# PersiaML/PERSIA

Measured on NVIDIA B200. Metric: samples/sec (Criteo-1TB-shape DLRM sparse path, 26 slots, dim128), higher is better.
Workload: dtype f32

## Files before the change

### persia_b200/csrc/pb_kernels.cuh

```cuda
#pragma once
#include <atomic>

#include "pb_common.cuh"

namespace pb {

struct SlotsDev {
  uint64_t prefix[PB_MAX_SLOTS];
  uint32_t occ_off[PB_MAX_SLOTS + 1];
  uint8_t sqrt_scaling[PB_MAX_SLOTS];
  uint32_t n_slots;
  uint64_t spacing;
  uint32_t spacing_bits;
  uint32_t uniform;
};

struct GradsDev {
  const void* ptr[PB_MAX_SLOTS];
  float inv_scale[PB_MAX_SLOTS];
  uint8_t do_scale[PB_MAX_SLOTS];
  const float* adam_pow;
  uint8_t pow_idx[PB_MAX_SLOTS];
};

constexpr uint32_t PB_GIANT_MIN = 1024;
constexpr uint32_t PB_HUGE_MIN = 256;
constexpr uint32_t PB_WARM_MAX = 32;
enum {
  BC_ITEMS = 0,
  BC_COLD,
  BC_WARM,
  BC_HOT,
  BC_SEG,
  BC_HUGE,
  BC_HOTW,
  BC_GIANT,
  BC_PEER = 8,
  BC_NEXT = 24,
  BC_COUNT = BC_NEXT + 2 * PB_MAX_SLOTS
};
struct BatchDev {
  DCell* set;
  uint32_t* occ_set;
  uint32_t* item_cell;
  uint32_t* seg_occ;
  uint2* cold;
  uint4* warm;
  uint4* hot;
  uint32_t* hot_bits;
  uint32_t hot_words;
  uint32_t hot_cap;
  uint32_t giant_cap;
  uint32_t* cnt;
  uint32_t n;
};

enum { XC_FLAG_SIGN = 0, XC_FLAG_ROW, XC_FLAG_GRAD, XC_COUNT, XC_WORDS };
constexpr uint32_t PB_MAX_RANKS = 16;
constexpr uint32_t PB_ADAM_KEYS = 256;
struct __align__(16) UCell {
  uint32_t row;
  uint32_t mask;
  uint32_t k[PB_MAX_RANKS];
  uint32_t pad[2];
};
struct XchgDev {
  uint64_t base[PB_MAX_RANKS];
  uint64_t off_sign, off_row, off_grad, off_gok;
  uint32_t R, rank, cap, row_f32;
  uint32_t* epoch;
  uint32_t* waited;
  uint32_t* own_row;
  uint32_t* own_cnt;
  uint32_t* err;
  UCell* ucell;
  uint32_t* uwin;
  uint32_t ucells;
  const uint64_t* akeys;
  uint32_t n_akeys;
  uint64_t amask;
  uint32_t* apresent;
  float* apow;
};

struct ReduceArgs {
  BatchDev b;
  const uint32_t* occ_outrow;
  const uint32_t* row_off;
  const uint32_t* tick_ptr;
  const uint32_t* nan_tick;
  float* vw_stage;
  uint32_t batch, round, quiet_miss;
  uint32_t round_mask[PB_MAX_SLOTS / 32];
  XchgDev x;
};

struct RawCell {
  uint64_t key;
  uint32_t first;
  uint32_t rank;
};
struct RawWork {
  RawCell* set;
  uint32_t set_mask;
  uint32_t* occ_set;
  uint32_t* flag;
  uint32_t* rank;
  uint32_t* tiles;
  uint32_t* distinct_cell;
  uint32_t* counts;
};

void launch_fill_cells(Cell* cells, uint64_t n, cudaStream_t st);
void launch_fill_set(DCell* set, uint64_t n, cudaStream_t st);
void launch_begin_batch(const TableDev& t, uint32_t* ctx_tick, uint32_t* batch_cnt, cudaStream_t st, bool bump = true);
void launch_probe(int mode, bool prefix, const TableDev& t, const HyperDev& hy, const OptimDev& op, const SlotsDev& sl,
                  const uint64_t* ids, uint32_t n, uint32_t* occ_cell, cudaStream_t st);
void launch_gather(const TableDev& t, const uint32_t* occ_cell, uint32_t n_out, float* out, cudaStream_t st);
void launch_dedup(const SlotsDev& sl, const BatchDev& b, const uint64_t* ids, cudaStream_t st);
void launch_probe_items(bool training, const TableDev& t, const HyperDev& hy, const OptimDev& op, const SlotsDev& sl,
                        const BatchDev& b, cudaStream_t st);
void launch_gather_items(const TableDev& t, const SlotsDev& sl, const BatchDev& b, const uint32_t* row_off,
// ... 72 lines not shown
```

### persia_b200/csrc/pb_reduce.cu

```cuda
#include <cstdlib>

#include "pb_optim.cuh"

namespace pb {

struct ItemSrc {
  const void* gbase;
  uint32_t slot_row0;
  float inv_scale;
  bool do_scale, do_sqrt, plain;
};

__device__ __forceinline__ ItemSrc item_src(const SlotsDev& sl, const GradsDev& gr, const ReduceArgs& a, uint32_t slot) {
  ItemSrc s;
  s.gbase = gr.ptr[slot];
  s.slot_row0 = slot * a.batch;
  s.inv_scale = gr.inv_scale[slot];
  s.do_scale = gr.do_scale[slot];
  s.do_sqrt = sl.sqrt_scaling[slot];
  s.plain = !a.occ_outrow && !s.do_scale && !s.do_sqrt;
  return s;
}

__device__ __forceinline__ uint32_t occ_out_row(const ReduceArgs& a, uint32_t occ) {
// ... 186 lines not shown
      } else {
        send_item<VEC, F16>(t, sl, gr, a, row, slot, cnt, lane, G, [&](uint32_t k) { return srt[k]; });
      }
      continue;
    }
    if (slot_dead(dead, slot)) continue;
    if (row >= t.capacity) {
      if (lane == 0 && !a.quiet_miss) atomicAdd(&t.counters[CTR_GRAD_MISS], 1u);
      continue;
    }
    float* stage = a.vw_stage ? a.vw_stage + (size_t)(n_cold + w) * t.dim : nullptr;
    step_item<VEC, F16, KIND>(t, op, hy, sl, gr, a, row, slot, cnt, lane, G, gmask, stage, [&](uint32_t k) { return srt[k]; });
  }
}

template <int VEC, bool F16, int KIND, bool SEND>
__global__ void __launch_bounds__(256) k_reduce_cold(TableDev t, OptimDev op, HyperDev hy, SlotsDev sl, GradsDev gr,
                                                     ReduceArgs a, uint32_t G) {
  __shared__ uint32_t dead[PB_MAX_SLOTS / 32];
  const uint32_t n_cold = a.b.cnt[BC_COLD];
  if (blockIdx.x * (blockDim.x / G) >= n_cold) return;
  build_dead_mask(dead, gr, a, sl.n_slots);
  const uint32_t lane = threadIdx.x % G, wl = threadIdx.x & 31;
  const uint32_t gmask = (G == 32) ? 0xffffffffu : (((1u << G) - 1u) << (wl / G * G));
  const uint32_t nvec = t.dim / VEC;
  for (uint32_t w = blockIdx.x * (blockDim.x / G) + threadIdx.x / G; w < n_cold; w += gridDim.x * (blockDim.x / G)) {
    const uint2 d = a.b.cold[w];
    const uint32_t slot = slot_of_occ(sl, d.y);
    const ItemSrc src = item_src(sl, gr, a, slot);
    const uint32_t orow = occ_out_row(a, d.y);
    const GradPrep prep = grad_prep(src, a, orow);
    const size_t gelem = (size_t)(orow - src.slot_row0) * t.dim;
    if (SEND) {
      if (d.x == ROW_NONE) continue;
      const bool off = slot_dead(dead, slot);
      if (lane == 0) *send_gok_ptr(a.x, d.x) = off ? 0u : 1u;
      if (off) continue;
      float* dst = send_grad_ptr(a.x, d.x, t.dim);
      for (uint32_t c = lane; c < nvec; c += G) {
        float g[VEC], acc[VEC];
        load_grad_elems<VEC, F16>(g, src.gbase, gelem, c * VEC);
#pragma unroll
        for (int q = 0; q < VEC; ++q) acc[q] = 0.0f;
        add_prepared<VEC>(acc, g, prep, src.plain);
        store_vec<VEC>(dst + c * VEC, acc);
      }
      continue;
    }
    if (slot_dead(dead, slot)) continue;
    if (d.x >= t.capacity) {
      if (lane == 0 && !a.quiet_miss) atomicAdd(&t.counters[CTR_GRAD_MISS], 1u);
      continue;
    }
    if (KIND == PB_OPT_ADAGRAD_VW) {
      const uint32_t occ = d.y;
      step_item<VEC, F16, KIND>(t, op, hy, sl, gr, a, d.x, slot, 1u, lane, G, gmask, a.vw_stage + (size_t)w * t.dim,
                                [&](uint32_t) { return occ; });
      continue;
    }
    float* prow = t.rows + (size_t)d.x * t.stride;
    StepCtx sc;
    sc.vw_state = sc.r1 = sc.r2 = 0.0f;
    if (KIND == PB_OPT_ADAM) sc = step_ctx(prow, t, op, gr, slot);
    for (uint32_t c = lane; c < nvec; c += G) {
      RowElems<KIND, VEC> rc;
      float g[VEC], acc[VEC];
      rc.load(prow, c * VEC, t, op);
      load_grad_elems<VEC, F16>(g, src.gbase, gelem, c * VEC);
#pragma unroll
      for (int q = 0; q < VEC; ++q) acc[q] = 0.0f;
      add_prepared<VEC>(acc, g, prep, src.plain);
      rc.step(c * VEC, acc, t, op, hy, sc);
      rc.store(prow, c * VEC, t, op);
    }
  }
}

constexpr uint32_t HOT_WIN = 8192;
constexpr uint32_t HOT_WORDS = HOT_WIN / 32;
constexpr uint32_t HOT_THREADS = 256;
constexpr uint32_t HOT_WARPS = HOT_THREADS / 32;
constexpr uint32_t HOT_MAX_SLOTS = 8;
constexpr uint32_t HOT_COLS = 512;
constexpr uint32_t WAIT_SPINS = 1u << 22;

__device__ __forceinline__ uint32_t smem_u32(const void* p) { return (uint32_t)__cvta_generic_to_shared(p); }
__device__ __forceinline__ void mbar_init(uint32_t bar, uint32_t count) {
  asm volatile("mbarrier.init.shared::cta.b64 [%0], %1;" ::"r"(bar), "r"(count) : "memory");
}
__device__ __forceinline__ void mbar_arrive(uint32_t bar) {
  asm volatile("mbarrier.arrive.shared::cta.b64 _, [%0];" ::"r"(bar) : "memory");
}
__device__ __forceinline__ bool mbar_wait(uint32_t bar, uint32_t parity) {
  for (uint32_t spins = 0; spins < WAIT_SPINS; ++spins) {
    uint32_t done;
    asm volatile(
        "{\n\t.reg .pred p;\n\t"
        "mbarrier.try_wait.parity.shared::cta.b64 p, [%1], %2;\n\t"
        "selp.u32 %0, 1, 0, p;\n\t}"
        : "=r"(done)
        : "r"(bar), "r"(parity)
        : "memory");
    if (done) return true;
  }
  return false;
}

__device__ __forceinline__ unsigned long long globaltimer_ns() {
  unsigned long long now;
  asm volatile("mov.u64 %0, %%globaltimer;" : "=l"(now));
  return now;
}
__device__ __forceinline__ bool mbar_test(uint32_t bar, uint32_t parity) {
  uint32_t done;
  asm volatile(
      "{\n\t.reg .pred p;\n\t"
      "mbarrier.test_wait.parity.shared::cta.b64 p, [%1], %2;\n\t"
      "selp.u32 %0, 1, 0, p;\n\t}"
      : "=r"(done)
      : "r"(bar), "r"(parity)
      : "memory");
  return done;
}

__device__ __forceinline__ __half2 clamp_h2(__half2 v) {
  const __half2 lim = __floats2half2_rn(65504.0f, 65504.0f);
  return __hmin2(__hmax2(v, __hneg2(lim)), lim);
}

struct HotGeom {
  uint32_t cols;
  uint32_t stride;
  uint32_t R;
  uint32_t R1;
  uint32_t S;
  uint32_t rowbytes;
  uint32_t lean;
  uint32_t CH;
  uint32_t vec;
  uint32_t vshift;
};

template <bool F16, bool POW2>
__device__ __forceinline__ void produce_vec(float* slot, const HotGeom& g, const ItemSrc& src, uint32_t my_row, float my_f,
                                            uint32_t nv, uint32_t col0, uint32_t dim, uint32_t lane) {
  constexpr uint32_t EV = F16 ? 8u : 4u;
  const unsigned char* gcol = reinterpret_cast<const unsigned char*>(src.gbase) + (size_t)col0 * (F16 ? 2u : 4u);
  const uint32_t rowbytes = dim * (F16 ? 2u : 4u);
  const uint32_t nvr = g.cols / EV, total = g.R1 * nvr, nv4 = (nv + 3u) & ~3u;
  uint4 raw[8];
#pragma unroll
  for (int j = 0; j < 8; ++j) {
    const uint32_t v = (uint32_t)j * 32u + lane;
    const uint32_t r = POW2 ? v >> g.vshift : v / nvr, c = POW2 ? v & (nvr - 1u) : v % nvr;
    const uint32_t grow = __shfl_sync(0xffffffffu, my_row, r & 31u);
    raw[j] = make_uint4(0u, 0u, 0u, 0u);
    if (v < total && r < nv) raw[j] = __ldg(reinterpret_cast<const uint4*>(gcol + (size_t)grow * rowbytes + c * 16u));
  }
  const bool prep = src.do_scale || src.do_sqrt;
#pragma unroll
  for (int j = 0; j < 8; ++j) {
    const uint32_t v = (uint32_t)j * 32u + lane;
    const uint32_t r = POW2 ? v >> g.vshift : v / nvr, c = POW2 ? v & (nvr - 1u) : v % nvr;
    float f = 1.0f;
    if (prep) f = __shfl_sync(0xffffffffu, my_f, r & 31u);
    if (v >= total || r >= nv4) continue;
    float x[EV];
    if constexpr (F16) {
      const __half2* h = reinterpret_cast<const __half2*>(&raw[j]);
#pragma unroll
      for (int q = 0; q < 4; ++q) {
        float2 y = __half22float2(clamp_h2(h[q]));
        x[2 * q] = y.x;
        x[2 * q + 1] = y.y;
      }
    } else {
      x[0] = __uint_as_float(raw[j].x); x[1] = __uint_as_float(raw[j].y);
      x[2] = __uint_as_float(raw[j].z); x[3] = __uint_as_float(raw[j].w);
    }
    if (prep) {
      if (src.do_scale) {
#pragma unroll
        for (uint32_t q = 0; q < EV; ++q) x[q] = __fmul_rn(x[q], src.inv_scale);
      }
      if (src.do_sqrt) {
#pragma unroll
        for (uint32_t q = 0; q < EV; ++q) x[q] = __fmul_rn(x[q], f);
      }
    }
    float4* dst = reinterpret_cast<float4*>(slot + (size_t)r * g.stride + c * EV);
    dst[0] = make_float4(x[0], x[1], x[2], x[3]);
    if constexpr (F16) dst[1] = make_float4(x[4], x[5], x[6], x[7]);
  }
}

template <bool F16>
__device__ __forceinline__ void produce_chunk(float* slot, const HotGeom& g, const ItemSrc& src, const ReduceArgs& a,
                                              const uint16_t* sorted, uint32_t k0, uint32_t nv, uint32_t wbase,
                                              uint32_t col0, uint32_t dim, uint32_t lane) {
  uint32_t my_row = 0;
  float my_f = 0.0f;
  if (lane < nv) {
    const uint32_t orow = occ_out_row(a, wbase + sorted[k0 + lane]);
    my_row = orow - src.slot_row0;
    my_f = src.do_sqrt ? grad_prep(src, a, orow).sqrt_f : 1.0f;
  }
  if (g.vec) {
    if (g.vshift < 32u) produce_vec<F16, true>(slot, g, src, my_row, my_f, nv, col0, dim, lane);
    else produce_vec<F16, false>(slot, g, src, my_row, my_f, nv, col0, dim, lane);
  } else {
    const unsigned char* gbytes = reinterpret_cast<const unsigned char*>(src.gbase);
    const uint32_t nv4 = min(g.R1, (nv + 3u) & ~3u), total = nv4 * g.cols;
    for (uint32_t i0 = 0; i0 < total; i0 += 32u) {
      const uint32_t i = i0 + lane;
      const bool ok = i < total;
      const uint32_t r = ok ? i / g.cols : 0u, c = ok ? i % g.cols : 0u;
      const uint32_t grow = __shfl_sync(0xffffffffu, my_row, r);
      const float f = __shfl_sync(0xffffffffu, my_f, r);
      if (!ok) continue;
      float x = 0.0f;
      if (r < nv) {
        const size_t e = (size_t)grow * dim + col0 + c;
        x = F16 ? clamp_f16(__half2float(reinterpret_cast<const __half*>(gbytes)[e])) : reinterpret_cast<const float*>(gbytes)[e];
        if (src.do_scale) x = __fmul_rn(x, src.inv_scale);
        if (src.do_sqrt) x = __fmul_rn(x, f);
      }
      slot[(size_t)r * g.stride + c] = x;
    }
  }
}

__device__ __forceinline__ void lean_load(uint4 (&raw)[8], const HotGeom& g, const unsigned char* gcol0, const uint16_t* sorted,
                                          uint32_t nv, uint32_t lane) {
  const uint32_t nvr_mask = (1u << g.vshift) - 1u;
  const uint32_t r0 = lane >> g.vshift, rstep = 32u >> g.vshift;
  const unsigned char* gc = gcol0 + (lane & nvr_mask) * 16u;
#pragma unroll
  for (int j = 0; j < 8; ++j) {
    const uint32_t r = (uint32_t)j * rstep + r0;
    raw[j] = make_uint4(0u, 0u, 0u, 0u);
    if (r < nv) raw[j] = __ldg(reinterpret_cast<const uint4*>(gc + (size_t)sorted[r] * g.rowbytes));
  }
}
template <bool F16>
__device__ __forceinline__ void lean_store(float* slot, const uint4 (&raw)[8], const HotGeom& g, uint32_t nv, uint32_t lane) {
  constexpr uint32_t EV = F16 ? 8u : 4u;
  const uint32_t nvr_mask = (1u << g.vshift) - 1u, nv4 = (nv + 3u) & ~3u;
  const uint32_t r0 = lane >> g.vshift, rstep = 32u >> g.vshift;
  float* sc = slot + (lane & nvr_mask) * EV;
#pragma unroll
  for (int j = 0; j < 8; ++j) {
    const uint32_t r = (uint32_t)j * rstep + r0;
    if (r >= nv4) continue;
    float4* dst = reinterpret_cast<float4*>(sc + (size_t)r * g.stride);
    if constexpr (F16) {
      const __half2* h = reinterpret_cast<const __half2*>(&raw[j]);
      const float2 y0 = __half22float2(clamp_h2(h[0])), y1 = __half22float2(clamp_h2(h[1]));
      const float2 y2 = __half22float2(clamp_h2(h[2])), y3 = __half22float2(clamp_h2(h[3]));
      dst[0] = make_float4(y0.x, y0.y, y1.x, y1.y);
      dst[1] = make_float4(y2.x, y2.y, y3.x, y3.y);
    } else {
      dst[0] = make_float4(__uint_as_float(raw[j].x), __uint_as_float(raw[j].y), __uint_as_float(raw[j].z), __uint_as_float(raw[j].w));
    }
  }
}

template <int EPL, int RB>
__device__ __forceinline__ void chain_block(float (&acc)[EPL], const float* rp, uint32_t stride) {
  float v[RB][EPL];
#pragma unroll
  for (int u = 0; u < RB; ++u) RowElems<-1, EPL>::template ld<EPL>(rp + (size_t)u * stride, v[u]);
#pragma unroll
  for (int u = 0; u < RB; ++u) {
#pragma unroll
    for (int q = 0; q < EPL; ++q) acc[q] = __fadd_rn(acc[q], v[u][q]);
  }
}

template <int EPL, bool F16, bool SEND>
__global__ void __launch_bounds__(HOT_THREADS, 1) k_reduce_hot(TableDev t, OptimDev op, HyperDev hy, SlotsDev sl, GradsDev gr,
                                                              ReduceArgs a, HotGeom geo, unsigned long long* trace) {
  extern __shared__ __align__(128) unsigned char smem_raw[];
  __shared__ uint32_t dead[PB_MAX_SLOTS / 32];
  __shared__ uint32_t s_item, s_nwin;
  __shared__ uint32_t bitmap[HOT_WORDS], wpre[HOT_WORDS];
  __shared__ uint16_t sorted[HOT_WIN];
  __shared__ __align__(8) uint64_t bars[2 * HOT_MAX_SLOTS];
  float* ring = reinterpret_cast<float*>(smem_raw);
  float* vstage = ring + (size_t)geo.S * geo.R * geo.stride;
  const uint32_t tid = threadIdx.x, warp = tid >> 5, lane = tid & 31;
  const uint32_t CH = geo.CH, PW = min(HOT_WARPS - CH, geo.S);
  if (tid == 0) {
    for (uint32_t s = 0; s < HOT_MAX_SLOTS; ++s) {
      mbar_init(smem_u32(bars + s), 32u);
      mbar_init(smem_u32(bars + HOT_MAX_SLOTS + s), 32u * CH);
    }
    asm volatile("fence.mbarrier_init.release.cluster;" ::: "memory");
  }
  build_dead_mask(dead, gr, a, sl.n_slots);
  const uint32_t full0 = smem_u32(bars), empty0 = smem_u32(bars + HOT_MAX_SLOTS);
  const uint32_t n_giant = a.b.cnt[BC_GIANT], n_huge = a.b.cnt[BC_HUGE];
  const uint32_t n_hot = a.b.cnt[BC_HOT] + n_huge + n_giant;
  uint32_t* next = a.b.cnt + BC_NEXT + PB_MAX_SLOTS + a.round;
  const uint32_t n_pass = (t.dim + HOT_COLS - 1u) / HOT_COLS;
  uint32_t it = 0;
  bool failed = false;
  for (;;) {
    __syncthreads();
    if (tid == 0) s_item = atomicAdd(next, 1u);
    __syncthreads();
    const uint32_t h = s_item;
    if (h >= n_hot) break;
    if (trace && tid == 0) trace[8 * h] = globaltimer_ns();
    const uint4 d = a.b.hot[h < n_giant ? a.b.hot_cap - 1u - h
                                        : (h < n_giant + n_huge ? a.b.hot_cap - 1u - a.b.giant_cap - (h - n_giant) : h - n_giant - n_huge)];
    const uint32_t row = d.x, cnt = d.z, slot = d.w;
    const bool bm_mode = d.y >> 31;
    const uint32_t base = d.y & 0x7FFFFFFFu;
    const uint32_t lo = sl.occ_off[slot], hi = sl.occ_off[slot + 1];
    bool skip = false;
    if (SEND) {
      skip = row == ROW_NONE || slot_dead(dead, slot);
      if (row != ROW_NONE && tid == 0) *send_gok_ptr(a.x, row) = slot_dead(dead, slot) ? 0u : 1u;
    } else {
      skip = slot_dead(dead, slot) || row >= t.capacity;
      if (!slot_dead(dead, slot) && row >= t.capacity && tid == 0 && !a.quiet_miss) atomicAdd(&t.counters[CTR_GRAD_MISS], 1u);
    }
    if (skip) {
      if (bm_mode)
        for (uint32_t w = tid; w < (hi - lo + 31u) / 32u; w += HOT_THREADS) a.b.hot_bits[base + w] = 0u;
      continue;
    }
    const ItemSrc src = item_src(sl, gr, a, slot);
    float* prow = SEND ? send_grad_ptr(a.x, row, t.dim) : t.rows + (size_t)row * t.stride;
    StepCtx sc;
    sc.vw_state = sc.r1 = sc.r2 = 0.0f;
    if (!SEND) sc = step_ctx(prow, t, op, gr, slot);
    for (uint32_t pass = 0; pass < n_pass; ++pass) {
      const uint32_t col0 = pass * HOT_COLS;
      HotGeom g = geo;
      g.cols = min(geo.cols, t.dim - col0);
      if (g.cols != geo.cols) g.vec = g.lean = 0;
      const bool lean = g.lean && src.plain;
      const uint32_t e0 = col0 + (warp * 32u + lane) * EPL;
      const bool own = warp < CH && e0 < t.dim;
      float acc[EPL];
#pragma unroll
      for (int q = 0; q < EPL; ++q) acc[q] = 0.0f;
      for (uint32_t wbase = lo; wbase < hi; wbase += HOT_WIN) {
        const uint32_t wend = min(hi, wbase + HOT_WIN);
        const uint32_t n_words = (wend - wbase + 31u) / 32u;
        if (bm_mode) {
          uint32_t* gw = a.b.hot_bits + base + (wbase - lo) / 32u;
          for (uint32_t w = tid; w < HOT_WORDS; w += HOT_THREADS) {
            bitmap[w] = w < n_words ? gw[w] : 0u;
            if (w < n_words && pass + 1 == n_pass) gw[w] = 0u;
          }
        } else {
          for (uint32_t w = tid; w < HOT_WORDS; w += HOT_THREADS) bitmap[w] = 0u;
          __syncthreads();
          for (uint32_t k0 = tid; k0 < cnt; k0 += 4 * HOT_THREADS) {
            uint32_t p[4];
#pragma unroll
            for (int u = 0; u < 4; ++u) p[u] = k0 + u * HOT_THREADS < cnt ? a.b.seg_occ[base + k0 + u * HOT_THREADS] : 0xFFFFFFFFu;
#pragma unroll
            for (int u = 0; u < 4; ++u)
              if (p[u] >= wbase && p[u] < wend) atomicOr(&bitmap[(p[u] - wbase) >> 5], 1u << ((p[u] - wbase) & 31u));
          }
        }
        __syncthreads();
        if (warp == 0) {
          uint32_t c[HOT_WORDS / 32], sum = 0;
#pragma unroll
          for (uint32_t j = 0; j < HOT_WORDS / 32; ++j) {
            c[j] = sum;
            sum += __popc(bitmap[lane * (HOT_WORDS / 32) + j]);
          }
          uint32_t inc = sum;
#pragma unroll
          for (int o = 1; o < 32; o <<= 1) {
            uint32_t y = __shfl_up_sync(0xffffffffu, inc, o);
            if (lane >= (uint32_t)o) inc += y;
          }
#pragma unroll
          for (uint32_t j = 0; j < HOT_WORDS / 32; ++j) wpre[lane * (HOT_WORDS / 32) + j] = inc - sum + c[j];
          if (lane == 31) s_nwin = inc;
        }
        __syncthreads();
        for (uint32_t w = tid; w < HOT_WORDS; w += HOT_THREADS) {
          uint32_t m = bitmap[w], at = wpre[w];
          while (m) {
            sorted[at++] = (uint16_t)(w * 32u + __ffs(m) - 1u);
            m &= m - 1u;
          }
        }
        __syncthreads();
        const uint32_t nwin = s_nwin;
        const uint32_t n_chunks = (nwin + g.R - 1u) / g.R;
        if (trace && tid == 0) trace[8 * h + 1] = globaltimer_ns();
        if (warp >= CH) {
          const uint32_t me = warp - CH;
          const unsigned char* gcol0 = reinterpret_cast<const unsigned char*>(src.gbase) +
                                       ((size_t)(wbase - src.slot_row0) * t.dim + col0) * (F16 ? 2u : 4u);
          for (uint32_t c = me < PW ? (me + PW - it % PW) % PW : n_chunks; c < n_chunks; c += PW) {
            const uint32_t i = it + c, stage = i % g.S, par = (i / g.S) & 1u;
            const uint32_t nv = min(g.R, nwin - c * g.R);
            float* slotp = ring + (size_t)stage * g.R * g.stride;
            const uint16_t* srt = sorted + c * g.R;
            if (lean) {
              uint4 ra[8], rb[8];
              const uint32_t np = (nv + g.R1 - 1u) / g.R1;
              lean_load(ra, g, gcol0, srt, min(g.R1, nv), lane);
              if (np > 1) lean_load(rb, g, gcol0, srt + g.R1, min(g.R1, nv - g.R1), lane);
              if (!failed && !mbar_wait(empty0 + 8u * stage, par ^ 1u)) failed = true;
              lean_store<F16>(slotp, ra, g, min(g.R1, nv), lane);
              if (np > 2) lean_load(ra, g, gcol0, srt + 2u * g.R1, min(g.R1, nv - 2u * g.R1), lane);
              if (np > 1) lean_store<F16>(slotp + (size_t)g.R1 * g.stride, rb, g, min(g.R1, nv - g.R1), lane);
              if (np > 3) lean_load(rb, g, gcol0, srt + 3u * g.R1, min(g.R1, nv - 3u * g.R1), lane);
              if (np > 2) lean_store<F16>(slotp + (size_t)2u * g.R1 * g.stride, ra, g, min(g.R1, nv - 2u * g.R1), lane);
              if (np > 3) lean_store<F16>(slotp + (size_t)3u * g.R1 * g.stride, rb, g, min(g.R1, nv - 3u * g.R1), lane);
            } else {
              if (!failed && !mbar_wait(empty0 + 8u * stage, par ^ 1u)) failed = true;
              for (uint32_t r0 = 0; r0 < nv; r0 += g.R1)
                produce_chunk<F16>(slotp + (size_t)r0 * g.stride, g, src, a, sorted, c * g.R + r0, min(g.R1, nv - r0), wbase, col0, t.dim, lane);
            }
            mbar_arrive(full0 + 8u * stage);
          }
        } else if (n_chunks) {
          long long tw = 0, ta = 0;
          for (uint32_t c = 0; c < n_chunks; ++c) {
            const uint32_t i = it + c;
            const uint32_t nv = min(g.R, nwin - c * g.R), stage = i % g.S, par = (i / g.S) & 1u;
            const long long c0 = trace ? clock64() : 0;
            if (!failed && !mbar_wait(full0 + 8u * stage, par)) failed = true;
            if (trace) { const long long c1 = clock64(); tw += c1 - c0; ta -= c1; }
            if (own) {
              const float* rp = ring + (size_t)stage * g.R * g.stride + (e0 - col0);
              if (nv == g.R && g.R == 64u) {
                chain_block<EPL, 32>(acc, rp, g.stride);
                chain_block<EPL, 32>(acc, rp + (size_t)32u * g.stride, g.stride);
              } else if (nv == g.R && g.R == 32u) {
                chain_block<EPL, 32>(acc, rp, g.stride);
              } else if (nv == g.R && g.R == 16u) {
                chain_block<EPL, 16>(acc, rp, g.stride);
              } else if (nv == g.R && g.R == 8u) {
                chain_block<EPL, 8>(acc, rp, g.stride);
              } else {
                for (uint32_t r = 0; r < nv; r += 4) chain_block<EPL, 4>(acc, rp + (size_t)r * g.stride, g.stride);
              }
            }
            mbar_arrive(empty0 + 8u * stage);
            if (trace) ta += clock64();
          }
          if (trace && tid == 0) { trace[8 * h + 4] = (unsigned long long)tw; trace[8 * h + 5] = (unsigned long long)ta; }
        }
        it += n_chunks;
      }
      if (trace && tid == 0) {
        trace[8 * h + 2] = globaltimer_ns();
        trace[8 * h + 3] = ((unsigned long long)blockIdx.x << 32) | cnt;
      }
      if (own) {
        const uint32_t nq = min((uint32_t)EPL, t.dim - e0);
        if (SEND) {
          if (nq == EPL) RowElems<-1, EPL>::template st<EPL>(prow + e0, acc);
          else for (uint32_t q = 0; q < nq; ++q) prow[e0 + q] = acc[q];
        } else if (nq == EPL) {
          RowElems<-1, EPL> rc;
          rc.load(prow, e0, t, op);
          if (op.kind == PB_OPT_ADAGRAD_VW) {
#pragma unroll
            for (int q = 0; q < EPL; ++q) vstage[e0 + q] = acc[q];
          }
          rc.step(e0, acc, t, op, hy, sc);
          rc.store(prow, e0, t, op);
        } else {
          for (uint32_t q = 0; q < nq; ++q) {
            RowElems<-1, 1> rc;
            float one[1] = {acc[q]};
            rc.load(prow, e0 + q, t, op);
            if (op.kind == PB_OPT_ADAGRAD_VW) vstage[e0 + q] = acc[q];
            rc.step(e0 + q, one, t, op, hy, sc);
            rc.store(prow, e0 + q, t, op);
          }
        }
      }
    }
    if (!SEND && op.kind == PB_OPT_ADAGRAD_VW) {
      __syncthreads();
      if (tid == 0) {
        float gs = __fdiv_rn(vw_dot(vstage, t.dim), (float)t.dim);
        prow[t.dim] = __fadd_rn(__fmul_rn(sc.vw_state, op.mom), gs);
      }
    }
  }
  if (failed && lane == 0) atomicAdd(&t.counters[CTR_ERR], 1u);
}

template <int VEC, bool F16>
static void items_dispatch(const TableDev& t, const OptimDev& op, const HyperDev& hy, const SlotsDev& sl, const GradsDev& gr,
                           const ReduceArgs& a, uint32_t G, cudaStream_t st, cudaStream_t st_warm, bool send) {
  const uint32_t per_block = 256u / G;
  uint32_t grid_cold = cdiv(a.b.n, per_block), grid_warm = cdiv(a.b.n / 2 + 1, per_block);
  if (grid_cold > 148u * 6u) grid_cold = 148u * 6u;
  if (grid_warm > 148u * 3u) grid_warm = 148u * 3u;
  if (send) {
    PB_LAUNCH_F(FAM_WARM, (k_reduce_warm<VEC, F16, PB_OPT_SGD, true>), grid_warm, 256, 0, st_warm, t, op, hy, sl, gr, a, G);
    PB_LAUNCH_F(FAM_UPDATE, (k_reduce_cold<VEC, F16, PB_OPT_SGD, true>), grid_cold, 256, 0, st, t, op, hy, sl, gr, a, G);
    return;
  }
#define PB_K(KK)                                                                                                   \
  case KK:                                                                                                         \
    PB_LAUNCH_F(FAM_WARM, (k_reduce_warm<VEC, F16, KK, false>), grid_warm, 256, 0, st_warm, t, op, hy, sl, gr, a, G); \
    PB_LAUNCH_F(FAM_UPDATE, (k_reduce_cold<VEC, F16, KK, false>), grid_cold, 256, 0, st, t, op, hy, sl, gr, a, G); \
    break;
  switch (op.kind) { PB_K(PB_OPT_SGD) PB_K(PB_OPT_ADAGRAD) PB_K(PB_OPT_ADAGRAD_VW) PB_K(PB_OPT_ADAM) }
#undef PB_K
}

static unsigned long long* g_hot_trace = nullptr;
void set_hot_trace(unsigned long long* p) { g_hot_trace = p; }

template <int EPL, bool F16, bool SEND>
static void hot_launch(const TableDev& t, const OptimDev& op, const HyperDev& hy, const SlotsDev& sl, const GradsDev& gr,
                       const ReduceArgs& a, uint32_t vec, cudaStream_t st) {
  HotGeom g;
  g.cols = t.dim < HOT_COLS ? t.dim : HOT_COLS;
  g.stride = (g.cols + 3u) & ~3u;
  g.CH = (g.cols + 32u * EPL - 1u) / (32u * EPL);
  g.rowbytes = t.dim * (F16 ? 2u : 4u);
  g.vec = vec;
  const uint32_t nvr = g.cols / (F16 ? 8u : 4u);
  g.vshift = 32u;
  if (vec && nvr && !(nvr & (nvr - 1u)))
    for (g.vshift = 0; (1u << g.vshift) < nvr; ++g.vshift) {}
  g.S = HOT_MAX_SLOTS;
  uint32_t slot_bytes = 8192;
  if (getenv("PB_HOT_SLOT_BYTES")) slot_bytes = (uint32_t)atoi(getenv("PB_HOT_SLOT_BYTES"));
  g.R = slot_bytes / (g.stride * 4u);
  if (g.R > 32u) g.R = 32u;
  if (vec && g.R * nvr > 256u) g.R = 256u / nvr;
  g.R &= ~3u;
  if (g.R < 4u) g.R = 4u;
  if (vec && g.R * nvr > 256u) g.vec = 0;
  g.lean = g.vec && g.vshift <= 5u && t.dim <= HOT_COLS && !a.occ_outrow && !getenv("PB_HOT_NO_LEAN");
  g.R1 = g.R;
  if (!getenv("PB_HOT_ONE_HALF")) {
    while (g.R < 64u && 2u * g.R * g.stride * 4u <= 32768u) g.R *= 2u;
    if (g.R * g.stride * 4u > 16384u) g.S = 6;
  }
  const size_t smem = (size_t)g.S * g.R * g.stride * 4u + (((size_t)t.dim + 3u) & ~(size_t)3u) * 4u;
  auto kern = k_reduce_hot<EPL, F16, SEND>;
  static size_t configured[64] = {0};
  int dev = 0;
  cudaGetDevice(&dev);
  if (dev >= 0 && dev < 64 && smem > configured[dev]) {
    cudaFuncSetAttribute(kern, cudaFuncAttributeMaxDynamicSharedMemorySize, (int)smem);
    configured[dev] = smem;
  }
  uint32_t per_sm = 1;
  if (getenv("PB_HOT_PER_SM")) per_sm = (uint32_t)atoi(getenv("PB_HOT_PER_SM"));
  const uint32_t cap_blocks = cdiv(a.b.n, PB_WARM_MAX + 1);
  uint32_t grid = 148u * per_sm;
  if (grid > cap_blocks) grid = cap_blocks ? cap_blocks : 1;
  PB_LAUNCH_F(FAM_HOT, kern, grid, HOT_THREADS, smem, st, t, op, hy, sl, gr, a, g, g_hot_trace);
}

void launch_reduce_items(const TableDev& t, const OptimDev& op, const HyperDev& hy, const SlotsDev& sl,
                         const GradsDev& gr, bool f16, const ReduceArgs& a, cudaStream_t st, cudaStream_t st_hot,
                         cudaStream_t st_warm, bool send) {
  if (!a.b.n) return;
  int vec, Gi;
  vec_group(t.dim, vec, Gi);
  uint32_t G = (uint32_t)Gi < 4u ? 4u : (uint32_t)Gi;
  {
    const uint32_t ev = f16 ? 8u : 4u;
    uint32_t hv = t.dim % ev == 0 ? 1u : 0u;
    for (uint32_t s = 0; s < sl.n_slots && hv; ++s)
      if (gr.ptr[s] && (reinterpret_cast<uintptr_t>(gr.ptr[s]) & 15u)) hv = 0;
    if (getenv("PB_HOT_NO_VEC")) hv = 0;
#define PB_H(E)                                                                 \
  if (send) {                                                                   \
    if (f16) hot_launch<E, true, true>(t, op, hy, sl, gr, a, hv, st_hot);       \
    else hot_launch<E, false, true>(t, op, hy, sl, gr, a, hv, st_hot);          \
  } else {                                                                      \
    if (f16) hot_launch<E, true, false>(t, op, hy, sl, gr, a, hv, st_hot);      \
    else hot_launch<E, false, false>(t, op, hy, sl, gr, a, hv, st_hot);         \
  }
    if (t.dim <= 128u && t.dim % 2u == 0) { PB_H(2) } else { PB_H(4) }
#undef PB_H
  }
  if (vec == 4) {
    if (f16) items_dispatch<4, true>(t, op, hy, sl, gr, a, G, st, st_warm, send);
    else items_dispatch<4, false>(t, op, hy, sl, gr, a, G, st, st_warm, send);
  } else {
    if (f16) items_dispatch<1, true>(t, op, hy, sl, gr, a, G, st, st_warm, send);
    else items_dispatch<1, false>(t, op, hy, sl, gr, a, G, st, st_warm, send);
  }
}

}
```

Before: 51.05 million.

## Rework hot-row gradient reduction with cp.async ring, raw-format staging, and giant-item column splitting

The hot reduce kernel now fills its shared-memory ring with cp.async plus mbarrier arrive instead of register loads followed by shared stores. Gradients are kept in their native format (f16 or f32) in the ring, and scale and sqrt factors are applied while the consumer warps accumulate. Giant items are split across U blocks by column range, with a per-item counter so the last block clears the hot bitmap. Ring geometry is rebuilt around larger slots (up to 128 rows) with two blocks per SM, and EPL=1 is used for dim≤128. This aims to raise memory-level parallelism and load balance for the few very large duplicate-id groups, at the cost of extra counters and a more complex synchronisation path.

After: 49.49 million, median of 6. 3.0% lower.

```diff
diff --git a/persia_b200/csrc/pb_kernels.cuh b/persia_b200/csrc/pb_kernels.cuh
--- a/persia_b200/csrc/pb_kernels.cuh
+++ b/persia_b200/csrc/pb_kernels.cuh
@@ -23,6 +23,7 @@
   uint8_t pow_idx[PB_MAX_SLOTS];
 };
 
+constexpr uint32_t PB_HOT_SPLIT_MAX = 32;
 constexpr uint32_t PB_GIANT_MIN = 1024;
 constexpr uint32_t PB_HUGE_MIN = 256;
 constexpr uint32_t PB_WARM_MAX = 32;
@@ -37,7 +38,8 @@
   BC_GIANT,
   BC_PEER = 8,
   BC_NEXT = 24,
-  BC_COUNT = BC_NEXT + 2 * PB_MAX_SLOTS
+  BC_SPLIT = BC_NEXT + 2 * PB_MAX_SLOTS,
+  BC_COUNT = BC_SPLIT + PB_HOT_SPLIT_MAX
 };
 struct BatchDev {
   DCell* set;
diff --git a/persia_b200/csrc/pb_reduce.cu b/persia_b200/csrc/pb_reduce.cu
--- a/persia_b200/csrc/pb_reduce.cu
+++ b/persia_b200/csrc/pb_reduce.cu
@@ -292,6 +292,9 @@
 constexpr uint32_t HOT_WARPS = HOT_THREADS / 32;
 constexpr uint32_t HOT_MAX_SLOTS = 8;
 constexpr uint32_t HOT_COLS = 512;
+constexpr uint32_t HOT_MAX_R = 128;
+constexpr uint32_t HOT_SLOT_BYTES = 32768;
+constexpr uint32_t HOT_RING_BYTES = 131072;
 constexpr uint32_t WAIT_SPINS = 1u << 22;
 
 __device__ __forceinline__ uint32_t smem_u32(const void* p) { return (uint32_t)__cvta_generic_to_shared(p); }
@@ -315,23 +318,18 @@
   }
   return false;
 }
+__device__ __forceinline__ void cp_async16(uint32_t dst, const void* src, uint32_t src_bytes) {
+  asm volatile("cp.async.cg.shared.global [%0], [%1], 16, %2;" ::"r"(dst), "l"(src), "r"(src_bytes) : "memory");
+}
+__device__ __forceinline__ void cp_async_mbar_arrive(uint32_t bar) {
+  asm volatile("cp.async.mbarrier.arrive.shared::cta.b64 [%0];" ::"r"(bar) : "memory");
+}
 
 __device__ __forceinline__ unsigned long long globaltimer_ns() {
   unsigned long long now;
   asm volatile("mov.u64 %0, %%globaltimer;" : "=l"(now));
   return now;
 }
-__device__ __forceinline__ bool mbar_test(uint32_t bar, uint32_t parity) {
-  uint32_t done;
-  asm volatile(
-      "{\n\t.reg .pred p;\n\t"
-      "mbarrier.test_wait.parity.shared::cta.b64 p, [%1], %2;\n\t"
-      "selp.u32 %0, 1, 0, p;\n\t}"
-      : "=r"(done)
-      : "r"(bar), "r"(parity)
-      : "memory");
-  return done;
-}
 
 __device__ __forceinline__ __half2 clamp_h2(__half2 v) {
   const __half2 lim = __floats2half2_rn(65504.0f, 65504.0f);
@@ -341,71 +339,30 @@
 struct HotGeom {
   uint32_t cols;
   uint32_t stride;
+  uint32_t slot_bytes;
   uint32_t R;
-  uint32_t R1;
   uint32_t S;
   uint32_t rowbytes;
-  uint32_t lean;
   uint32_t CH;
   uint32_t vec;
-  uint32_t vshift;
+  uint32_t U;
 };
 
-template <bool F16, bool POW2>
-__device__ __forceinline__ void produce_vec(float* slot, const HotGeom& g, const ItemSrc& src, uint32_t my_row, float my_f,
-                                            uint32_t nv, uint32_t col0, uint32_t dim, uint32_t lane) {
-  constexpr uint32_t EV = F16 ? 8u : 4u;
-  const unsigned char* gcol = reinterpret_cast<const unsigned char*>(src.gbase) + (size_t)col0 * (F16 ? 2u : 4u);
-  const uint32_t rowbytes = dim * (F16 ? 2u : 4u);
-  const uint32_t nvr = g.cols / EV, total = g.R1 * nvr, nv4 = (nv + 3u) & ~3u;
-  uint4 raw[8];
-#pragma unroll
-  for (int j = 0; j < 8; ++j) {
-    const uint32_t v = (uint32_t)j * 32u + lane;
-    const uint32_t r = POW2 ? v >> g.vshift : v / nvr, c = POW2 ? v & (nvr - 1u) : v % nvr;
-    const uint32_t grow = __shfl_sync(0xffffffffu, my_row, r & 31u);
-    raw[j] = make_uint4(0u, 0u, 0u, 0u);
-    if (v < total && r < nv) raw[j] = __ldg(reinterpret_cast<const uint4*>(gcol + (size_t)grow * rowbytes + c * 16u));
-  }
-  const bool prep = src.do_scale || src.do_sqrt;
-#pragma unroll
-  for (int j = 0; j < 8; ++j) {
-    const uint32_t v = (uint32_t)j * 32u + lane;
-    const uint32_t r = POW2 ? v >> g.vshift : v / nvr, c = POW2 ? v & (nvr - 1u) : v % nvr;
-    float f = 1.0f;
-    if (prep) f = __shfl_sync(0xffffffffu, my_f, r & 31u);
-    if (v >= total || r >= nv4) continue;
-    float x[EV];
-    if constexpr (F16) {
-      const __half2* h = reinterpret_cast<const __half2*>(&raw[j]);
-#pragma unroll
-      for (int q = 0; q < 4; ++q) {
-        float2 y = __half22float2(clamp_h2(h[q]));
-        x[2 * q] = y.x;
-        x[2 * q + 1] = y.y;
-      }
-    } else {
-      x[0] = __uint_as_float(raw[j].x); x[1] = __uint_as_float(raw[j].y);
-      x[2] = __uint_as_float(raw[j].z); x[3] = __uint_as_float(raw[j].w);
-    }
-    if (prep) {
-      if (src.do_scale) {
-#pragma unroll
-        for (uint32_t q = 0; q < EV; ++q) x[q] = __fmul_rn(x[q], src.inv_scale);
-      }
-      if (src.do_sqrt) {
-#pragma unroll
-        for (uint32_t q = 0; q < EV; ++q) x[q] = __fmul_rn(x[q], f);
-      }
-    }
-    float4* dst = reinterpret_cast<float4*>(slot + (size_t)r * g.stride + c * EV);
-    dst[0] = make_float4(x[0], x[1], x[2], x[3]);
-    if constexpr (F16) dst[1] = make_float4(x[4], x[5], x[6], x[7]);
+template <bool POW2>
+__device__ __forceinline__ void copy_chunk(uint32_t slot, const unsigned char* gcol, const ItemSrc& src, const ReduceArgs& a,
+                                           const uint16_t* srt, uint32_t nv, uint32_t wbase, uint32_t nvr, uint32_t vshift,
+                                           uint32_t ring_rowbytes, uint32_t rowbytes, uint32_t lane) {
+  const uint32_t total = ((nv + 3u) & ~3u) * nvr;
+  for (uint32_t v = lane; v < total; v += 32u) {
+    const uint32_t r = POW2 ? v >> vshift : v / nvr, c = v - r * nvr;
+    const bool live = r < nv;
+    const uint32_t grow = live ? occ_out_row(a, wbase + srt[r]) - src.slot_row0 : 0u;
+    cp_async16(slot + r * ring_rowbytes + c * 16u, gcol + (size_t)grow * rowbytes + c * 16u, live ? 16u : 0u);
   }
 }
 
 template <bool F16>
-__device__ __forceinline__ void produce_chunk(float* slot, const HotGeom& g, const ItemSrc& src, const ReduceArgs& a,
+__device__ __forceinline__ void produce_chunk(float* slot, const HotGeom& g, uint32_t cols, const ItemSrc& src, const ReduceArgs& a,
                                               const uint16_t* sorted, uint32_t k0, uint32_t nv, uint32_t wbase,
                                               uint32_t col0, uint32_t dim, uint32_t lane) {
   uint32_t my_row = 0;
@@ -415,91 +372,113 @@
     my_row = orow - src.slot_row0;
     my_f = src.do_sqrt ? grad_prep(src, a, orow).sqrt_f : 1.0f;
   }
-  if (g.vec) {
-    if (g.vshift < 32u) produce_vec<F16, true>(slot, g, src, my_row, my_f, nv, col0, dim, lane);
-    else produce_vec<F16, false>(slot, g, src, my_row, my_f, nv, col0, dim, lane);
-  } else {
-    const unsigned char* gbytes = reinterpret_cast<const unsigned char*>(src.gbase);
-    const uint32_t nv4 = min(g.R1, (nv + 3u) & ~3u), total = nv4 * g.cols;
-    for (uint32_t i0 = 0; i0 < total; i0 += 32u) {
-      const uint32_t i = i0 + lane;
-      const bool ok = i < total;
-      const uint32_t r = ok ? i / g.cols : 0u, c = ok ? i % g.cols : 0u;
-      const uint32_t grow = __shfl_sync(0xffffffffu, my_row, r);
-      const float f = __shfl_sync(0xffffffffu, my_f, r);
-      if (!ok) continue;
-      float x = 0.0f;
-      if (r < nv) {
-        const size_t e = (size_t)grow * dim + col0 + c;
-        x = F16 ? clamp_f16(__half2float(reinterpret_cast<const __half*>(gbytes)[e])) : reinterpret_cast<const float*>(gbytes)[e];
-        if (src.do_scale) x = __fmul_rn(x, src.inv_scale);
-        if (src.do_sqrt) x = __fmul_rn(x, f);
-      }
-      slot[(size_t)r * g.stride + c] = x;
-    }
-  }
-}
-
-__device__ __forceinline__ void lean_load(uint4 (&raw)[8], const HotGeom& g, const unsigned char* gcol0, const uint16_t* sorted,
-                                          uint32_t nv, uint32_t lane) {
-  const uint32_t nvr_mask = (1u << g.vshift) - 1u;
-  const uint32_t r0 = lane >> g.vshift, rstep = 32u >> g.vshift;
-  const unsigned char* gc = gcol0 + (lane & nvr_mask) * 16u;
-#pragma unroll
-  for (int j = 0; j < 8; ++j) {
-    const uint32_t r = (uint32_t)j * rstep + r0;
-    raw[j] = make_uint4(0u, 0u, 0u, 0u);
-    if (r < nv) raw[j] = __ldg(reinterpret_cast<const uint4*>(gc + (size_t)sorted[r] * g.rowbytes));
-  }
-}
-template <bool F16>
-__device__ __forceinline__ void lean_store(float* slot, const uint4 (&raw)[8], const HotGeom& g, uint32_t nv, uint32_t lane) {
-  constexpr uint32_t EV = F16 ? 8u : 4u;
-  const uint32_t nvr_mask = (1u << g.vshift) - 1u, nv4 = (nv + 3u) & ~3u;
-  const uint32_t r0 = lane >> g.vshift, rstep = 32u >> g.vshift;
-  float* sc = slot + (lane & nvr_mask) * EV;
-#pragma unroll
-  for (int j = 0; j < 8; ++j) {
-    const uint32_t r = (uint32_t)j * rstep + r0;
-    if (r >= nv4) continue;
-    float4* dst = reinterpret_cast<float4*>(sc + (size_t)r * g.stride);
-    if constexpr (F16) {
-      const __half2* h = reinterpret_cast<const __half2*>(&raw[j]);
-      const float2 y0 = __half22float2(clamp_h2(h[0])), y1 = __half22float2(clamp_h2(h[1]));
-      const float2 y2 = __half22float2(clamp_h2(h[2])), y3 = __half22float2(clamp_h2(h[3]));
-      dst[0] = make_float4(y0.x, y0.y, y1.x, y1.y);
-      dst[1] = make_float4(y2.x, y2.y, y3.x, y3.y);
+  const unsigned char* gbytes = reinterpret_cast<const unsigned char*>(src.gbase);
+  const uint32_t nv4 = min(32u, (nv + 3u) & ~3u), total = nv4 * cols;
+  for (uint32_t i0 = 0; i0 < total; i0 += 32u) {
+    const uint32_t i = i0 + lane;
+    const bool ok = i < total;
+    const uint32_t r = ok ? i / cols : 0u, c = ok ? i % cols : 0u;
+    const uint32_t grow = __shfl_sync(0xffffffffu, my_row, r);
+    const float f = __shfl_sync(0xffffffffu, my_f, r);
+    if (!ok) continue;
+    float x = 0.0f;
+    if (r < nv) {
+      const size_t e = (size_t)grow * dim + col0 + c;
+      x = F16 ? clamp_f16(__half2float(reinterpret_cast<const __half*>(gbytes)[e])) : reinterpret_cast<const float*>(gbytes)[e];
+      if (src.do_scale) x = __fmul_rn(x, src.inv_scale);
+      if (src.do_sqrt) x = __fmul_rn(x, f);
+    }
+    slot[(size_t)r * g.stride + c] = x;
+  }
+}
+
+template <int EPL, bool H>
+struct RingElems {
+  static constexpr int W = H ? (EPL + 1) / 2 : EPL;
+  uint32_t w[W];
+  __device__ __forceinline__ void ld(const void* p) {
+    if constexpr (H && EPL == 1) {
+      w[0] = *reinterpret_cast<const unsigned short*>(p);
+    } else if constexpr (W == 1) {
+      w[0] = *reinterpret_cast<const uint32_t*>(p);
+    } else if constexpr (W == 2) {
+      const uint2 t = *reinterpret_cast<const uint2*>(p);
+      w[0] = t.x; w[1] = t.y;
     } else {
-      dst[0] = make_float4(__uint_as_float(raw[j].x), __uint_as_float(raw[j].y), __uint_as_float(raw[j].z), __uint_as_float(raw[j].w));
-    }
-  }
-}
-
-template <int EPL, int RB>
-__device__ __forceinline__ void chain_block(float (&acc)[EPL], const float* rp, uint32_t stride) {
-  float v[RB][EPL];
-#pragma unroll
-  for (int u = 0; u < RB; ++u) RowElems<-1, EPL>::template ld<EPL>(rp + (size_t)u * stride, v[u]);
+      static_assert(W == 4, "EPL");
+      const uint4 t = *reinterpret_cast<const uint4*>(p);
+      w[0] = t.x; w[1] = t.y; w[2] = t.z; w[3] = t.w;
+    }
+  }
+  __device__ __forceinline__ void get(float (&x)[EPL]) const {
+    if constexpr (H && EPL == 1) {
+      x[0] = clamp_f16(__half2float(__ushort_as_half((unsigned short)w[0])));
+    } else if constexpr (H) {
+#pragma unroll
+      for (int q = 0; q < W; ++q) {
+        const float2 y = __half22float2(clamp_h2(*reinterpret_cast<const __half2*>(&w[q])));
+        x[2 * q] = y.x; x[2 * q + 1] = y.y;
+      }
+    } else {
+#pragma unroll
+      for (int q = 0; q < EPL; ++q) x[q] = __uint_as_float(w[q]);
+    }
+  }
+};
+
+template <int EPL, bool H, bool PREP, int RB>
+__device__ __forceinline__ void chain_block(float (&acc)[EPL], const unsigned char* rp, uint32_t row_bytes, const float* rf, float s) {
+  RingElems<EPL, H> v[RB];
+#pragma unroll
+  for (int u = 0; u < RB; ++u) v[u].ld(rp + (size_t)u * row_bytes);
 #pragma unroll
   for (int u = 0; u < RB; ++u) {
-#pragma unroll
-    for (int q = 0; q < EPL; ++q) acc[q] = __fadd_rn(acc[q], v[u][q]);
-  }
+    float x[EPL];
+    v[u].get(x);
+    if (PREP) {
+      const float f = rf[u];
+#pragma unroll
+      for (int q = 0; q < EPL; ++q) x[q] = __fmul_rn(__fmul_rn(x[q], s), f);
+    }
+#pragma unroll
+    for (int q = 0; q < EPL; ++q) acc[q] = __fadd_rn(acc[q], x[q]);
+  }
+}
+
+template <int EPL, bool H, bool PREP>
+__device__ __forceinline__ void chain_chunk(float (&acc)[EPL], const unsigned char* rp, uint32_t row_bytes, const float* rf, float s,
+                                            uint32_t nv, uint32_t R) {
+  constexpr uint32_t RB = RingElems<EPL, H>::W > 2 ? 16u : 32u;
+  if (nv == R && R == 128u) {
+#pragma unroll
+    for (uint32_t k = 0; k < 128u; k += RB) chain_block<EPL, H, PREP, RB>(acc, rp + k * row_bytes, row_bytes, rf + k, s);
+    return;
+  }
+  if (nv == R && R == 64u) {
+#pragma unroll
+    for (uint32_t k = 0; k < 64u; k += RB) chain_block<EPL, H, PREP, RB>(acc, rp + k * row_bytes, row_bytes, rf + k, s);
+    return;
+  }
+  uint32_t r = 0;
+  for (; r + RB <= nv; r += RB) chain_block<EPL, H, PREP, RB>(acc, rp + (size_t)r * row_bytes, row_bytes, rf + r, s);
+  for (; r < nv; r += 4u) chain_block<EPL, H, PREP, 4>(acc, rp + (size_t)r * row_bytes, row_bytes, rf + r, s);
 }
 
 template <int EPL, bool F16, bool SEND>
-__global__ void __launch_bounds__(HOT_THREADS, 1) k_reduce_hot(TableDev t, OptimDev op, HyperDev hy, SlotsDev sl, GradsDev gr,
+__global__ void __launch_bounds__(HOT_THREADS, 2) k_reduce_hot(TableDev t, OptimDev op, HyperDev hy, SlotsDev sl, GradsDev gr,
                                                               ReduceArgs a, HotGeom geo, unsigned long long* trace) {
   extern __shared__ __align__(128) unsigned char smem_raw[];
   __shared__ uint32_t dead[PB_MAX_SLOTS / 32];
-  __shared__ uint32_t s_item, s_nwin;
+  __shared__ uint32_t s_item, s_nwin, s_last;
   __shared__ uint32_t bitmap[HOT_WORDS], wpre[HOT_WORDS];
   __shared__ uint16_t sorted[HOT_WIN];
   __shared__ __align__(8) uint64_t bars[2 * HOT_MAX_SLOTS];
-  float* ring = reinterpret_cast<float*>(smem_raw);
-  float* vstage = ring + (size_t)geo.S * geo.R * geo.stride;
+  unsigned char* ring = smem_raw;
+  float* rowf = reinterpret_cast<float*>(ring + (size_t)geo.S * geo.slot_bytes);
+  float* vstage = rowf + (size_t)geo.S * geo.R;
   const uint32_t tid = threadIdx.x, warp = tid >> 5, lane = tid & 31;
   const uint32_t CH = geo.CH, PW = min(HOT_WARPS - CH, geo.S);
+  constexpr uint32_t ESZ = F16 ? 2u : 4u;
   if (tid == 0) {
     for (uint32_t s = 0; s < HOT_MAX_SLOTS; ++s) {
       mbar_init(smem_u32(bars + s), 32u);
@@ -511,6 +490,7 @@
   const uint32_t full0 = smem_u32(bars), empty0 = smem_u32(bars + HOT_MAX_SLOTS);
   const uint32_t n_giant = a.b.cnt[BC_GIANT], n_huge = a.b.cnt[BC_HUGE];
   const uint32_t n_hot = a.b.cnt[BC_HOT] + n_huge + n_giant;
+  const uint32_t U = geo.U, n_split = U > 1u ? min(n_giant, PB_HOT_SPLIT_MAX) : 0u, n_units = n_hot + n_split * (U - 1u);
   uint32_t* next = a.b.cnt + BC_NEXT + PB_MAX_SLOTS + a.round;
   const uint32_t n_pass = (t.dim + HOT_COLS - 1u) / HOT_COLS;
   uint32_t it = 0;
@@ -519,8 +499,10 @@
     __syncthreads();
     if (tid == 0) s_item = atomicAdd(next, 1u);
     __syncthreads();
-    const uint32_t h = s_item;
-    if (h >= n_hot) break;
+    const uint32_t hu = s_item;
+    if (hu >= n_units) break;
+    const bool split = hu < n_split * U;
+    const uint32_t h = split ? hu / U : hu - n_split * (U - 1u), part = split ? hu % U : 0u;
     if (trace && tid == 0) trace[8 * h] = globaltimer_ns();
     const uint4 d = a.b.hot[h < n_giant ? a.b.hot_cap - 1u - h
                                         : (h < n_giant + n_huge ? a.b.hot_cap - 1u - a.b.giant_cap - (h - n_giant) : h - n_giant - n_huge)];
@@ -531,10 +513,10 @@
     bool skip = false;
     if (SEND) {
       skip = row == ROW_NONE || slot_dead(dead, slot);
-      if (row != ROW_NONE && tid == 0) *send_gok_ptr(a.x, row) = slot_dead(dead, slot) ? 0u : 1u;
+      if (row != ROW_NONE && tid == 0 && part == 0) *send_gok_ptr(a.x, row) = slot_dead(dead, slot) ? 0u : 1u;
     } else {
       skip = slot_dead(dead, slot) || row >= t.capacity;
-      if (!slot_dead(dead, slot) && row >= t.capacity && tid == 0 && !a.quiet_miss) atomicAdd(&t.counters[CTR_GRAD_MISS], 1u);
+      if (!slot_dead(dead, slot) && row >= t.capacity && tid == 0 && part == 0 && !a.quiet_miss) atomicAdd(&t.counters[CTR_GRAD_MISS], 1u);
     }
     if (skip) {
       if (bm_mode)
@@ -542,18 +524,16 @@
       continue;
     }
     const ItemSrc src = item_src(sl, gr, a, slot);
+    const float scale = src.do_scale ? src.inv_scale : 1.0f;
     float* prow = SEND ? send_grad_ptr(a.x, row, t.dim) : t.rows + (size_t)row * t.stride;
     StepCtx sc;
     sc.vw_state = sc.r1 = sc.r2 = 0.0f;
     if (!SEND) sc = step_ctx(prow, t, op, gr, slot);
-    for (uint32_t pass = 0; pass < n_pass; ++pass) {
-      const uint32_t col0 = pass * HOT_COLS;
-      HotGeom g = geo;
-      g.cols = min(geo.cols, t.dim - col0);
-      if (g.cols != geo.cols) g.vec = g.lean = 0;
-      const bool lean = g.lean && src.plain;
+    for (uint32_t pass = 0; pass < (split ? 1u : n_pass); ++pass) {
+      const uint32_t col0 = split ? part * (t.dim / U) : pass * HOT_COLS;
+      const uint32_t cols = split ? t.dim / U : min(geo.cols, t.dim - col0), cend = col0 + cols;
       const uint32_t e0 = col0 + (warp * 32u + lane) * EPL;
-      const bool own = warp < CH && e0 < t.dim;
+      const bool own = warp < CH && e0 < cend;
       float acc[EPL];
 #pragma unroll
       for (int q = 0; q < EPL; ++q) acc[q] = 0.0f;
@@ -564,7 +544,7 @@
           uint32_t* gw = a.b.hot_bits + base + (wbase - lo) / 32u;
           for (uint32_t w = tid; w < HOT_WORDS; w += HOT_THREADS) {
             bitmap[w] = w < n_words ? gw[w] : 0u;
-            if (w < n_words && pass + 1 == n_pass) gw[w] = 0u;
+            if (w < n_words && pass + 1 == n_pass && !split) gw[w] = 0u;
           }
         } else {
           for (uint32_t w = tid; w < HOT_WORDS; w += HOT_THREADS) bitmap[w] = 0u;
@@ -606,33 +586,34 @@
         }
         __syncthreads();
         const uint32_t nwin = s_nwin;
-        const uint32_t n_chunks = (nwin + g.R - 1u) / g.R;
+        const uint32_t n_chunks = (nwin + geo.R - 1u) / geo.R;
         if (trace && tid == 0) trace[8 * h + 1] = globaltimer_ns();
         if (warp >= CH) {
           const uint32_t me = warp - CH;
-          const unsigned char* gcol0 = reinterpret_cast<const unsigned char*>(src.gbase) +
-                                       ((size_t)(wbase - src.slot_row0) * t.dim + col0) * (F16 ? 2u : 4u);
+          const unsigned char* gcol = reinterpret_cast<const unsigned char*>(src.gbase) + (size_t)col0 * ESZ;
+          const uint32_t nvr = cols * ESZ / 16u, vshift = __ffs(nvr) - 1u;
+          const uint32_t ring_rowbytes = geo.stride * (geo.vec ? ESZ : 4u);
           for (uint32_t c = me < PW ? (me + PW - it % PW) % PW : n_chunks; c < n_chunks; c += PW) {
-            const uint32_t i = it + c, stage = i % g.S, par = (i / g.S) & 1u;
-            const uint32_t nv = min(g.R, nwin - c * g.R);
-            float* slotp = ring + (size_t)stage * g.R * g.stride;
-            const uint16_t* srt = sorted + c * g.R;
-            if (lean) {
-              uint4 ra[8], rb[8];
-              const uint32_t np = (nv + g.R1 - 1u) / g.R1;
-              lean_load(ra, g, gcol0, srt, min(g.R1, nv), lane);
-              if (np > 1) lean_load(rb, g, gcol0, srt + g.R1, min(g.R1, nv - g.R1), lane);
-              if (!failed && !mbar_wait(empty0 + 8u * stage, par ^ 1u)) failed = true;
-              lean_store<F16>(slotp, ra, g, min(g.R1, nv), lane);
-              if (np > 2) lean_load(ra, g, gcol0, srt + 2u * g.R1, min(g.R1, nv - 2u * g.R1), lane);
-              if (np > 1) lean_store<F16>(slotp + (size_t)g.R1 * g.stride, rb, g, min(g.R1, nv - g.R1), lane);
-              if (np > 3) lean_load(rb, g, gcol0, srt + 3u * g.R1, min(g.R1, nv - 3u * g.R1), lane);
-              if (np > 2) lean_store<F16>(slotp + (size_t)2u * g.R1 * g.stride, ra, g, min(g.R1, nv - 2u * g.R1), lane);
-              if (np > 3) lean_store<F16>(slotp + (size_t)3u * g.R1 * g.stride, rb, g, min(g.R1, nv - 3u * g.R1), lane);
+            const uint32_t i = it + c, stage = i % geo.S, par = (i / geo.S) & 1u;
+            const uint32_t nv = min(geo.R, nwin - c * geo.R);
+            unsigned char* slotp = ring + (size_t)stage * geo.slot_bytes;
+            const uint16_t* srt = sorted + c * geo.R;
+            if (!failed && !mbar_wait(empty0 + 8u * stage, par ^ 1u)) failed = true;
+            if (geo.vec) {
+              if (!src.plain) {
+                float* rf = rowf + (size_t)stage * geo.R;
+                for (uint32_t r = lane; r < ((nv + 3u) & ~3u); r += 32u)
+                  rf[r] = r < nv && src.do_sqrt ? grad_prep(src, a, occ_out_row(a, wbase + srt[r])).sqrt_f : 1.0f;
+              }
+              if (nvr & (nvr - 1u))
+                copy_chunk<false>(smem_u32(slotp), gcol, src, a, srt, nv, wbase, nvr, vshift, ring_rowbytes, geo.rowbytes, lane);
+              else
+                copy_chunk<true>(smem_u32(slotp), gcol, src, a, srt, nv, wbase, nvr, vshift, ring_rowbytes, geo.rowbytes, lane);
+              cp_async_mbar_arrive(full0 + 8u * stage);
             } else {
-              if (!failed && !mbar_wait(empty0 + 8u * stage, par ^ 1u)) failed = true;
-              for (uint32_t r0 = 0; r0 < nv; r0 += g.R1)
-                produce_chunk<F16>(slotp + (size_t)r0 * g.stride, g, src, a, sorted, c * g.R + r0, min(g.R1, nv - r0), wbase, col0, t.dim, lane);
+              for (uint32_t r0 = 0; r0 < nv; r0 += 32u)
+                produce_chunk<F16>(reinterpret_cast<float*>(slotp) + (size_t)r0 * geo.stride, geo, cols, src, a, sorted,
+                                   c * geo.R + r0, min(32u, nv - r0), wbase, col0, t.dim, lane);
             }
             mbar_arrive(full0 + 8u * stage);
           }
@@ -640,24 +621,19 @@
           long long tw = 0, ta = 0;
           for (uint32_t c = 0; c < n_chunks; ++c) {
             const uint32_t i = it + c;
-            const uint32_t nv = min(g.R, nwin - c * g.R), stage = i % g.S, par = (i / g.S) & 1u;
+            const uint32_t nv = min(geo.R, nwin - c * geo.R), stage = i % geo.S, par = (i / geo.S) & 1u;
             const long long c0 = trace ? clock64() : 0;
             if (!failed && !mbar_wait(full0 + 8u * stage, par)) failed = true;
             if (trace) { const long long c1 = clock64(); tw += c1 - c0; ta -= c1; }
             if (own) {
-              const float* rp = ring + (size_t)stage * g.R * g.stride + (e0 - col0);
-              if (nv == g.R && g.R == 64u) {
-                chain_block<EPL, 32>(acc, rp, g.stride);
-                chain_block<EPL, 32>(acc, rp + (size_t)32u * g.stride, g.stride);
-              } else if (nv == g.R && g.R == 32u) {
-                chain_block<EPL, 32>(acc, rp, g.stride);
-              } else if (nv == g.R && g.R == 16u) {
-                chain_block<EPL, 16>(acc, rp, g.stride);
-              } else if (nv == g.R && g.R == 8u) {
-                chain_block<EPL, 8>(acc, rp, g.stride);
-              } else {
-                for (uint32_t r = 0; r < nv; r += 4) chain_block<EPL, 4>(acc, rp + (size_t)r * g.stride, g.stride);
-              }
+              const unsigned char* slotp = ring + (size_t)stage * geo.slot_bytes;
+              const float* rf = rowf + (size_t)stage * geo.R;
+              if (!geo.vec)
+                chain_chunk<EPL, false, false>(acc, slotp + (e0 - col0) * 4u, geo.stride * 4u, rf, 1.0f, nv, geo.R);
+              else if (src.plain)
+                chain_chunk<EPL, F16, false>(acc, slotp + (e0 - col0) * ESZ, geo.stride * ESZ, rf, 1.0f, nv, geo.R);
+              else
+                chain_chunk<EPL, F16, true>(acc, slotp + (e0 - col0) * ESZ, geo.stride * ESZ, rf, scale, nv, geo.R);
             }
             mbar_arrive(empty0 + 8u * stage);
             if (trace) ta += clock64();
@@ -671,7 +647,7 @@
         trace[8 * h + 3] = ((unsigned long long)blockIdx.x << 32) | cnt;
       }
       if (own) {
-        const uint32_t nq = min((uint32_t)EPL, t.dim - e0);
+        const uint32_t nq = min((uint32_t)EPL, cend - e0);
         if (SEND) {
           if (nq == EPL) RowElems<-1, EPL>::template st<EPL>(prow + e0, acc);
           else for (uint32_t q = 0; q < nq; ++q) prow[e0 + q] = acc[q];
@@ -694,6 +670,15 @@
             rc.store(prow, e0 + q, t, op);
           }
         }
+      }
+    }
+    if (split && bm_mode) {
+      __syncthreads();
+      if (tid == 0) s_last = atomicAdd(&a.b.cnt[BC_SPLIT + h], 1u) == U - 1u;
+      __syncthreads();
+      if (s_last) {
+        for (uint32_t w = tid; w < (hi - lo + 31u) / 32u; w += HOT_THREADS) a.b.hot_bits[base + w] = 0u;
+        if (tid == 0) a.b.cnt[BC_SPLIT + h] = 0u;
       }
     }
     if (!SEND && op.kind == PB_OPT_ADAGRAD_VW) {
@@ -736,30 +721,26 @@
                        const ReduceArgs& a, uint32_t vec, cudaStream_t st) {
   HotGeom g;
   g.cols = t.dim < HOT_COLS ? t.dim : HOT_COLS;
-  g.stride = (g.cols + 3u) & ~3u;
   g.CH = (g.cols + 32u * EPL - 1u) / (32u * EPL);
   g.rowbytes = t.dim * (F16 ? 2u : 4u);
   g.vec = vec;
-  const uint32_t nvr = g.cols / (F16 ? 8u : 4u);
-  g.vshift = 32u;
-  if (vec && nvr && !(nvr & (nvr - 1u)))
-    for (g.vshift = 0; (1u << g.vshift) < nvr; ++g.vshift) {}
-  g.S = HOT_MAX_SLOTS;
-  uint32_t slot_bytes = 8192;
-  if (getenv("PB_HOT_SLOT_BYTES")) slot_bytes = (uint32_t)atoi(getenv("PB_HOT_SLOT_BYTES"));
-  g.R = slot_bytes / (g.stride * 4u);
-  if (g.R > 32u) g.R = 32u;
-  if (vec && g.R * nvr > 256u) g.R = 256u / nvr;
+  g.U = 1u;
+  {
+    uint32_t u = 2u;
+    if (getenv("PB_HOT_SPLIT")) u = (uint32_t)atoi(getenv("PB_HOT_SPLIT"));
+    if (u > 1u && vec && op.kind != PB_OPT_ADAGRAD_VW && t.dim <= HOT_COLS && t.dim % (u * (F16 ? 8u : 4u)) == 0) g.U = u;
+  }
+  g.stride = vec ? g.cols : (g.cols + 3u) & ~3u;
+  const uint32_t ring_rowbytes = g.stride * (vec && F16 ? 2u : 4u);
+  g.R = HOT_SLOT_BYTES / ring_rowbytes;
+  if (g.R > HOT_MAX_R) g.R = HOT_MAX_R;
   g.R &= ~3u;
   if (g.R < 4u) g.R = 4u;
-  if (vec && g.R * nvr > 256u) g.vec = 0;
-  g.lean = g.vec && g.vshift <= 5u && t.dim <= HOT_COLS && !a.occ_outrow && !getenv("PB_HOT_NO_LEAN");
-  g.R1 = g.R;
-  if (!getenv("PB_HOT_ONE_HALF")) {
-    while (g.R < 64u && 2u * g.R * g.stride * 4u <= 32768u) g.R *= 2u;
-    if (g.R * g.stride * 4u > 16384u) g.S = 6;
-  }
-  const size_t smem = (size_t)g.S * g.R * g.stride * 4u + (((size_t)t.dim + 3u) & ~(size_t)3u) * 4u;
+  g.slot_bytes = g.R * ring_rowbytes;
+  g.S = HOT_RING_BYTES / g.slot_bytes;
+  if (g.S > HOT_MAX_SLOTS) g.S = HOT_MAX_SLOTS;
+  if (g.S < 1u) g.S = 1u;
+  const size_t smem = (size_t)g.S * g.slot_bytes + (size_t)g.S * g.R * 4u + (((size_t)t.dim + 3u) & ~(size_t)3u) * 4u;
   auto kern = k_reduce_hot<EPL, F16, SEND>;
   static size_t configured[64] = {0};
   int dev = 0;
@@ -797,7 +778,7 @@
     if (f16) hot_launch<E, true, false>(t, op, hy, sl, gr, a, hv, st_hot);      \
     else hot_launch<E, false, false>(t, op, hy, sl, gr, a, hv, st_hot);         \
   }
-    if (t.dim <= 128u && t.dim % 2u == 0) { PB_H(2) } else { PB_H(4) }
+    if (t.dim <= 128u) { PB_H(1) } else { PB_H(4) }
 #undef PB_H
   }
   if (vec == 4) {
```
